# LuxGraph/Lux

Hardware: AMD Instinct MI355X
Metric: GTEPS (higher is better)
Workload: dtype fp32; 1 GPU; model=pagerank, graph=rmat27, nv=134217728, ne=2147483648, parallelism=graph-partition x1

## Files before the change

lux_amd/_native_gpu.py:

```python
import ctypes
import os

_DIR = os.path.dirname(os.path.abspath(__file__))
_PATH = os.path.join(_DIR, "liblux_gpu.so")

_lib = None


def lib():
    global _lib
    if _lib is None:
        if not os.path.exists(_PATH):
            raise RuntimeError(
                "liblux_gpu.so not built — run `python build.py --gpu` "
                "(the HIP extension is mandatory on GPU boxes; no fallback)")
        _lib = ctypes.CDLL(_PATH)
        _lib.lux_gpu_scan_partials_size.restype = ctypes.c_uint32
    return _lib


def dp(t):
    if t is None:
        return ctypes.c_void_p(0)
    if isinstance(t, int):
# ... 104 lines not shown
    lib().lux_gpu_build_bitmap(_u64(stream), _u32(vp), dp(snapshot),
                               dp(new_labels), dp(seg))


def d2s(stream, vp, row_left, dense_seg, sparse_seg):
    lib().lux_gpu_d2s(_u64(stream), _u32(vp), _u32(row_left), dp(dense_seg),
                      dp(sparse_seg))


def check(stream, is_min, vp, row_left, row_ptr_loc, col, labels, mistakes):
    lib().lux_gpu_check(_u64(stream), ctypes.c_int(is_min), _u32(vp),
                        _u32(row_left), dp(row_ptr_loc), dp(col), dp(labels),
                        dp(mistakes))


PULL_PR = 0
PULL_MIN = 1
PULL_MAX = 2


def pull_iter(stream, mode, n0, bin0, n1, bin1, n2, bin2, nbig, bin2v,
              row_ptr, col, oldv, newv, deg, row_left, init_rank,
              row_u32=0):
    lib().lux_gpu_pull_iter(_u64(stream), ctypes.c_int(mode), _u32(n0),
                            dp(bin0), _u32(n1), dp(bin1), _u32(n2), dp(bin2),
                            _u32(nbig), dp(bin2v), dp(row_ptr),
                            ctypes.c_int(row_u32), dp(col),
                            dp(oldv), dp(newv), dp(deg), _u32(row_left),
                            ctypes.c_float(init_rank))


def blocked_count(stream, ep, col, row_ptr_loc, vp, bounds, nb, counts,
                  lo=0, hi=0xFFFFFFFF):
    lib().lux_gpu_blocked_count(_u64(stream), _u64(ep), dp(col),
                                dp(row_ptr_loc), _u32(vp), dp(bounds),
                                ctypes.c_int(nb), _u32(lo), _u32(hi),
                                dp(counts))


def blocked_scatter(stream, ep, col, row_ptr_loc, vp, bounds, nb, cursor,
                    out_col, lo=0, hi=0xFFFFFFFF):
    lib().lux_gpu_blocked_scatter(_u64(stream), _u64(ep), dp(col),
                                  dp(row_ptr_loc), _u32(vp), dp(bounds),
                                  ctypes.c_int(nb), _u32(lo), _u32(hi),
                                  dp(cursor), dp(out_col))


def pull_finish_pr(stream, vp, newv, deg, row_left, init_rank):
    lib().lux_gpu_pull_finish_pr(_u64(stream), _u32(vp), dp(newv), dp(deg),
                                 _u32(row_left), ctypes.c_float(init_rank))


def pull_active_flags(stream, vp, row_ptr, flags):
    lib().lux_gpu_pull_active_flags(_u64(stream), _u32(vp), dp(row_ptr),
                                    dp(flags))


def pull_active_list(stream, vp, flags, ends, active):
    lib().lux_gpu_pull_active_list(_u64(stream), _u32(vp), dp(flags),
                                   dp(ends), dp(active))


def pull_build_slots(stream, n, bin_, row_ptr, row_u32, ends, cidx, rng):
    lib().lux_gpu_pull_build_slots(_u64(stream), _u32(n), dp(bin_),
                                   dp(row_ptr), ctypes.c_int(row_u32),
                                   dp(ends), dp(cidx), dp(rng))


def pull_build_hub_slots(stream, n2, bin2, row_ptr, row_u32, ends, cidx,
                         rng):
    lib().lux_gpu_pull_build_hub_slots(_u64(stream), _u32(n2), dp(bin2),
                                       dp(row_ptr), ctypes.c_int(row_u32),
                                       dp(ends), dp(cidx), dp(rng))


def pull_slots_iter(stream, n0, cidx0, rng0, n1, cidx1, rng1, n2, cidx2,
                    rng2, col, oldv, acc):
    lib().lux_gpu_pull_slots_iter(_u64(stream), _u32(n0), dp(cidx0),
                                  dp(rng0), _u32(n1), dp(cidx1), dp(rng1),
                                  _u32(n2), dp(cidx2), dp(rng2), dp(col),
                                  dp(oldv), dp(acc))


def pull_finish_pr_active(stream, na, active, acc, out, deg, row_left,
                          init_rank):
    lib().lux_gpu_pull_finish_pr_active(_u64(stream), _u32(na), dp(active),
                                        dp(acc), dp(out), dp(deg),
                                        _u32(row_left),
                                        ctypes.c_float(init_rank))


def pull_fill_inactive_pr(stream, vp, row_ptr, out, deg, row_left,
                          init_rank):
    lib().lux_gpu_pull_fill_inactive_pr(_u64(stream), _u32(vp), dp(row_ptr),
                                        dp(out), dp(deg), _u32(row_left),
                                        ctypes.c_float(init_rank))


def cf_als_iter(stream, n0, bin0, n1, bin1, n2, bin2, nbig, bin2v, hubidx,
                gram_scratch, rhs_scratch, row_ptr, col, w, oldv, newv,
                row_left, K, oldv_bf=None):
    lib().lux_gpu_cf_als_iter(
        _u64(stream), _u32(n0), dp(bin0), _u32(n1), dp(bin1), _u32(n2),
        dp(bin2), _u32(nbig), dp(bin2v), dp(hubidx), dp(gram_scratch),
        dp(rhs_scratch), dp(row_ptr), dp(col), dp(w), dp(oldv), dp(oldv_bf),
        dp(newv), _u32(row_left), ctypes.c_int(K))


def frontier_expand(stream, old_dense, in_row_left, in_count, old_seg,
                    qlabels, labels_repair, push_row_ptr, items, counter,
                    max_items):
    lib().lux_gpu_frontier_expand(
        _u64(stream), ctypes.c_int(old_dense), _u32(in_row_left),
        _u32(in_count), dp(old_seg), dp(qlabels), dp(labels_repair),
        dp(push_row_ptr), dp(items), dp(counter), _u32(max_items))


def frontier_expand_auto(stream, verts, in_row_left, seg, qlabels,
                         labels_repair, push_row_ptr, items, counter,
                         max_items):
    lib().lux_gpu_frontier_expand_auto(
        _u64(stream), _u32(verts), _u32(in_row_left), dp(seg), dp(qlabels),
        dp(labels_repair), dp(push_row_ptr), dp(items), dp(counter),
        _u32(max_items))


def frontier_fixup(stream, vp, row_left, capacity, built_dense, snapshot,
                   labels_part, deg_part, new_seg, annex, tmp_seg, meta,
                   item_counter, max_items):
    lib().lux_gpu_frontier_fixup(
        _u64(stream), _u32(vp), _u32(row_left), _u32(capacity),
        ctypes.c_int(built_dense), dp(snapshot), dp(labels_part),
        dp(deg_part), dp(new_seg), dp(annex), dp(tmp_seg), dp(meta),
        dp(item_counter), _u32(max_items))


def push_chunk_scatter(stream, is_min, new_dense, items, counter, max_items,
                       push_row_ptr, push_col, old_labels, snapshot,
                       new_labels, my_row_left, new_seg, capacity,
                       visited_bits=None):
    lib().lux_gpu_push_chunk_scatter(
        _u64(stream), ctypes.c_int(is_min), ctypes.c_int(new_dense),
        dp(items), dp(counter), _u32(max_items), dp(push_row_ptr),
        dp(push_col), dp(old_labels), dp(snapshot), dp(new_labels),
        _u32(my_row_left), dp(new_seg), _u32(capacity), dp(visited_bits))


def publish_labels_guarded(stream, vp, meta, labels_part, labels_slice):
    lib().lux_gpu_publish_labels_guarded(_u64(stream), _u32(vp), dp(meta),
                                         dp(labels_part), dp(labels_slice))


def bits_from_labels(stream, vp, labels, bits):
    lib().lux_gpu_bits_from_labels(_u64(stream), _u32(vp), dp(labels),
                                   dp(bits))


def uf_union_star(stream, nv, star, parent):
    lib().lux_gpu_uf_union_star(_u64(stream), _u32(nv), dp(star), dp(parent))


def uf_flatten(stream, nv, parent, labels):
    lib().lux_gpu_uf_flatten(_u64(stream), _u32(nv), dp(parent), dp(labels))


def uf_union_binned(stream, n0, bin0, n1, bin1, n2, bin2, row_ptr, col,
# ... 16 lines not shown
```

lux_amd/engine.py:

```python

import torch

from . import _native_gpu as ng
from . import dist as dx

U32 = torch.int32
U64 = torch.int64
F32 = torch.float32


def _stream():
    return torch.cuda.current_stream().cuda_stream


LLC_BLOCK_SHIFT = 23


def _bins_for(row_ptr, vp, ep, device, compact=False):
    s = _stream()
    bin0 = torch.empty(max(vp, 1), dtype=U32, device=device)
    bin1 = torch.empty(max(vp, 1), dtype=U32, device=device)
    nbig_max = max(min(vp, ep // 2048 + 1), 1)
    n2_max = ep // 8192 + nbig_max + 1
    bin2 = torch.empty(n2_max * 2, dtype=U32, device=device)
    bin2v = torch.empty(nbig_max, dtype=U32, device=device)
    counters = torch.zeros(4, dtype=U32, device=device)
    ng.build_bins(s, vp, row_ptr, bin0, bin1, bin2, bin2v, counters)
    c = counters.cpu()
    n0, n1, n2, nbig = int(c[0]), int(c[1]), int(c[2]), int(c[3])
    if compact:
        bin0 = bin0[:max(n0, 1)].clone()
        bin1 = bin1[:max(n1, 1)].clone()
        bin2 = bin2[:max(n2 * 2, 1)].clone()
        bin2v = bin2v[:max(nbig, 1)].clone()
    return n0, n1, n2, nbig, bin0, bin1, bin2, bin2v


def run_pull_sweeps(part, mode, oldv, newv, deg, init_rank, subset=None):
    s = _stream()
    blocks = getattr(part, "blocks", None)
    if blocks:
        for blk in blocks:
            if subset == "local" and not blk["local"]:
                continue
            if subset == "remote" and blk["local"]:
                continue
            if isinstance(subset, tuple) and subset[0] == "peer" \
                    and blk.get("owner") != subset[1]:
                continue
            ng.pull_iter(s, mode, blk["n0"], blk["bin0"], blk["n1"],
                         blk["bin1"], blk["n2"], blk["bin2"], blk["nbig"],
                         blk["bin2v"], blk["row_ptr"], blk["col"], oldv,
                         newv, deg, part.row_left, init_rank,
                         row_u32=blk.get("row_u32", 0))
    else:
        assert subset is None, "subset sweeps need the blocked CSC"
        ng.pull_iter(s, mode, part.n0, part.bin0, part.n1, part.bin1,
                     part.n2, part.bin2, part.nbig, part.bin2v, part.row_ptr,
                     part.col, oldv, newv, deg, part.row_left, init_rank)


def run_pull_slots_sweeps(part, oldv, acc):
    s = _stream()
    for src in part.slot_srcs:
        ng.pull_slots_iter(s, src["n0"], src["cidx0"], src["rng0"],
                           src["n1"], src["cidx1"], src["rng1"], src["n2"],
                           src["cidx2"], src["rng2"], src["col"], oldv, acc)


def seed_pull(part, mode, oldv, newv):
    if mode == ng.PULL_PR:
        newv.zero_()
    else:
        newv.copy_(oldv.narrow(0, part.row_left, part.vp))


def run_pull(part, mode, oldv, newv, deg, init_rank, seed=True):
    if seed:
        seed_pull(part, mode, oldv, newv)
    run_pull_sweeps(part, mode, oldv, newv, deg, init_rank)
    if mode == ng.PULL_PR:
        ng.pull_finish_pr(_stream(), part.vp, newv, deg, part.row_left,
                          init_rank)


def partition_bounds(col_end, ne, nparts):
    nv = col_end.numel()
    cap = (ne + nparts - 1) // nparts
    targets = torch.tensor(
        [min(cap * (p + 1), ne) for p in range(nparts)], dtype=U64,
        device=col_end.device)
    cuts = torch.searchsorted(col_end, targets, right=True)
    cuts = cuts.cpu().tolist()
    row_left, row_right = [], []
    v = 0
    for p in range(nparts):
        rl = v
        rr = max(cuts[p] - 1, rl) if p < nparts - 1 else nv - 1
        rr = min(rr, nv - 1)
        if rl >= nv:
            row_left.append(1)
            row_right.append(0)
            continue
        row_left.append(rl)
        row_right.append(rr)
        v = rr + 1
    return row_left, row_right


class DeviceCSC:

    n_users = None

    def __init__(self, nv, ne, col_end, src, weight=None):
        self.nv, self.ne = nv, ne
        self.col_end, self.src, self.weight = col_end, src, weight

    @classmethod
    def rmat(cls, scale, ne, seed=1, device="cuda", sym=False):
        nv = 1 << scale
        s = _stream()
        npairs = ne // 2 if sym else ne
        esrc = torch.empty(npairs, dtype=U32, device=device)
        edst = torch.empty(npairs, dtype=U32, device=device)
        ng.rmat_edges(s, seed, scale, npairs, esrc, edst)
        if sym:
            esrc, edst = (torch.cat([esrc, edst]), torch.cat([edst, esrc]))
        g = cls._from_device_edges(nv, npairs * 2 if sym else ne, esrc,
                                   edst, None, device)
        return g

    @classmethod
    def rmat_folded(cls, nv, ne, seed=1, device="cuda", sym=False):
        scale = 0
        while (1 << scale) < nv:
            scale += 1
        s = _stream()
        npairs = ne // 2 if sym else ne
        esrc = torch.empty(npairs, dtype=U32, device=device)
        edst = torch.empty(npairs, dtype=U32, device=device)
        ng.rmat_edges_folded(s, seed, scale, nv, npairs, esrc, edst)
        if sym:
            esrc, edst = (torch.cat([esrc, edst]), torch.cat([edst, esrc]))
        return cls._from_device_edges(nv, npairs * 2 if sym else ne, esrc,
                                      edst, None, device)

# ... 213 lines not shown
            return
        (self.n0, self.n1, self.n2, self.nbig, self.bin0, self.bin1,
         self.bin2, self.bin2v) = _bins_for(self.row_ptr, self.vp, self.ep,
                                            self.device)

    def pull_bounds(self, shift):
        bounds = set(range(0, self.nv, 1 << shift)) | {self.nv}
        if self.nparts > 1 and self.vp > 0:
            for q in range(self.nparts):
                if self.verts_all[q]:
                    bounds |= {self.row_left_all[q],
                               self.row_right_all[q] + 1}
        return sorted(bounds)

    def prepare_pull(self, force_shift=None):
        self.build_bins()
        if getattr(self, "blocks", None) is not None:
            return
        shift = force_shift if force_shift is not None else int(
            __import__("os").environ.get("LUX_BLOCK_SHIFT", LLC_BLOCK_SHIFT))
        if force_shift is None and torch.cuda.is_available() \
                and self.vp > 0:
            free, _total = torch.cuda.mem_get_info(self.device)
            while shift < 30:
                sb = len(self.pull_bounds(shift)) - 1
                need = 12 * sb * self.vp + 4 * self.ep
                if need < free * 0.85:
                    break
                shift += 1
        bounds = self.pull_bounds(shift)
        if self.ep == 0 or len(bounds) <= 2:
            self.blocks = None
            return
        if force_shift is None and self.nv <= (1 << shift) \
                and self.nparts == 1:
            self.blocks = None
            return
        self.build_blocked(bounds)

    def prepare_pull_slots(self):
        if getattr(self, "slot_srcs", None) is not None:
            return True
        self.prepare_pull()
        if not self.blocks and self.ep >= (1 << 32):
            return False
        device, s, vp = self.device, _stream(), self.vp
        before = torch.cuda.memory_allocated(device)
        self.na = 0
        self.active = torch.empty(1, dtype=U32, device=device)
        self.slot_srcs = []
        if vp == 0 or self.ep == 0:
            self.slot_bytes = 0
            return True
        flags = torch.empty(vp, dtype=U32, device=device)
        ng.pull_active_flags(s, vp, self.row_ptr, flags)
        ends = torch.empty(vp, dtype=U64, device=device)
        partials = torch.empty(ng.scan_partials_size(vp), dtype=U64,
                               device=device)
        ng.scan_end_offsets(s, vp, flags, ends, partials)
        self.na = int(ends[vp - 1].item())
        self.active = torch.empty(max(self.na, 1), dtype=U32, device=device)
        ng.pull_active_list(s, vp, flags, ends, self.active)
        if self.blocks:
            srcs = self.blocks
        else:
            srcs = [dict(row_ptr=self.row_ptr, row_u32=0, col=self.col,
                         n0=self.n0, n1=self.n1, n2=self.n2, bin0=self.bin0,
                         bin1=self.bin1, bin2=self.bin2)]
        for src in srcs:
            for k, build in (("0", ng.pull_build_slots),
                             ("1", ng.pull_build_slots),
                             ("2", ng.pull_build_hub_slots)):
                n = src["n" + k]
                cidx = torch.empty(max(n, 1), dtype=U32, device=device)
                rng = torch.empty(max(2 * n, 2), dtype=U32, device=device)
                build(s, n, src["bin" + k], src["row_ptr"],
                      src.get("row_u32", 0), ends, cidx, rng)
                src["cidx" + k], src["rng" + k] = cidx, rng
            self.slot_srcs.append(src)
        torch.cuda.synchronize()
        del flags, ends, partials
        self.slot_bytes = torch.cuda.memory_allocated(device) - before
        return True

    def build_blocked(self, bounds):
        import os
        device = self.device
        s = _stream()
        vp, ep = self.vp, self.ep
        sb = len(bounds) - 1
        cap = int(os.environ.get("LUX_BLOCK_GROUP_SLOTS", "0") or 0)
        if not cap and torch.cuda.is_available():
            free, _total = torch.cuda.mem_get_info(device)
            cap = int(max(free - 4 * ep - (2 << 30), 1 << 30) * 0.85) // 12
        bpg = sb if not cap else max(1, min(sb, cap // max(vp, 1)))
        blk_col = torch.empty(max(ep, 1), dtype=U32, device=device)
        self.blocks = []
        global_begin = 0
        for g0 in range(0, sb, bpg):
            g1 = min(sb, g0 + bpg)
            nb = g1 - g0
            slots = nb * vp
            bounds_g = torch.tensor(bounds[g0:g1 + 1], dtype=U32,
                                    device=device)
            counts = torch.zeros(slots, dtype=U32, device=device)
            ng.blocked_count(s, ep, self.col, self.row_ptr, vp, bounds_g,
                             nb + 1, counts, lo=bounds[g0], hi=bounds[g1])
            cursor = torch.zeros(slots + 1, dtype=U64, device=device)
            partials = torch.empty(ng.scan_partials_size(slots), dtype=U64,
                                   device=device)
            ng.scan_end_offsets(s, slots, counts,
                                cursor.narrow(0, 1, slots), partials)
            torch.cuda.synchronize()
            del counts, partials
            torch.cuda.empty_cache()
            if global_begin:
                cursor += global_begin
            ng.blocked_scatter(s, ep, self.col, self.row_ptr, vp, bounds_g,
                               nb + 1, cursor.narrow(0, 0, slots), blk_col,
                               lo=bounds[g0], hi=bounds[g1])
            ends = cursor.narrow(0, 0, slots)
            begin = global_begin
            for b in range(nb):
                end = int(ends[(b + 1) * vp - 1].item())
                if end == begin:
                    continue
                row_ptr_b = torch.empty(vp + 1, dtype=U64, device=device)
                ng.local_row_ptr(s, vp, begin, ends.narrow(0, b * vp, vp),
                                 row_ptr_b)
                col_b = blk_col.narrow(0, begin, end - begin)
                n0, n1, n2, nbig, b0, b1, b2, b2v = _bins_for(
                    row_ptr_b, vp, end - begin, device, compact=True)
                row32 = torch.empty(vp + 1, dtype=U32, device=device)
                ng.u64_to_u32(s, vp + 1, row_ptr_b, row32)
                del row_ptr_b
                gb = g0 + b
                owner = -1
                if self.nparts > 1:
                    for q in range(self.nparts):
                        if self.verts_all[q] \
                                and bounds[gb] >= self.row_left_all[q] \
                                and bounds[gb + 1] \
                                <= self.row_right_all[q] + 1:
                            owner = q
                            break
                local = self.nparts > 1 and owner == self.p
                self.blocks.append(dict(row_ptr=row32, row_u32=1, col=col_b,
                                        n0=n0, n1=n1, n2=n2, nbig=nbig,
                                        bin0=b0, bin1=b1, bin2=b2,
                                        bin2v=b2v, local=local,
                                        owner=owner))
                begin = end
            global_begin = int(ends[slots - 1].item())
            del ends, cursor
        self._blk_col = blk_col


def _maybe_halo(part):
    if dx.world_size() <= 1 or part.vp == 0:
        return None
    from .halo import HaloExchange
    h = HaloExchange(part.nv, part.row_left_all, part.verts_all, part.p,
                     part.col)
    return h if h.worth_it() else None


def _publish_async(engine, my_slice):
    p = engine.part
    if engine.halo is not None:
        return engine.halo.publish_async(engine.old, my_slice)
    return dx.all_gather_slices_async(engine.old, my_slice, p.verts_all,
                                      p.row_left_all, my_index=p.p)


def _wait_handle(engine):
    h = engine._handle
    engine._handle = None
    if h is None:
        return
    if isinstance(h, list):
        for _q, w in h:
            w.wait()
    else:
        h.wait()


def _finalize_full(engine):
    _wait_handle(engine)
    if engine.halo is None:
        return
    p = engine.part
    dx.all_gather_slices(engine.old,
                         engine.old.narrow(0, p.row_left, p.vp),
                         p.verts_all, p.row_left_all, my_index=p.p)


class PagerankEngine:

    def __init__(self, part: GraphPart):
        self.part = part
        device = part.device
        s = _stream()
        deg = torch.zeros(part.nv, dtype=U32, device=device)
        ng.hist_u32(s, part.ep, part.col, deg)
        dx.all_reduce_sum_(deg)
        self.deg = deg
        part.prepare_pull()
        rank0 = 1.0 / part.nv
        degf = deg.to(F32)
        self.old = torch.where(deg == 0, torch.full_like(degf, rank0),
                               rank0 / degf.clamp(min=1.0))
        self.init_rank = (1.0 - 0.15) / part.nv
        import os
        self._slots = (dx.world_size() == 1
                       and os.environ.get("LUX_PULL_SLOTS", "1") != "0"
                       and part.prepare_pull_slots())
        if self._slots:
            self.acc = torch.empty(max(part.na, 1), dtype=F32,
                                   device=device)
            self.new_part = None
            self._inactive_done = False
        else:
            self.new_part = torch.empty(part.vp, dtype=F32, device=device)
        self.cur_part = self.old.narrow(0, part.row_left,
                                        part.vp).clone()
        self._handle = None
        self.halo = _maybe_halo(part)
        self._graph = None
        self._steps = 0

    def _pipelined(self):
        p = self.part
        return dx.world_size() > 1 and p.blocks is not None and p.vp > 0

    def _step_body(self):
        p = self.part
        if self._slots:
            self.acc.zero_()
            run_pull_slots_sweeps(p, self.old, self.acc)
            ng.pull_finish_pr_active(_stream(), p.na, p.active, self.acc,
                                     self.old, self.deg, p.row_left,
                                     self.init_rank)
            return
        run_pull(p, ng.PULL_PR, self.old, self.new_part, self.deg,
                 self.init_rank)
        self.old.narrow(0, p.row_left, p.vp).copy_(self.new_part)

    def _step_single(self):
        import os
        if self._graph is not None:
            self._graph.replay()
            return
        if self._steps >= 2 and os.environ.get("LUX_HIPGRAPH", "1") \
                == "1" and not os.environ.get("LUX_SYNC_CHECK"):
            try:
                g = torch.cuda.CUDAGraph()
                with torch.cuda.graph(g):
                    self._step_body()
                self._graph = g
                self._graph.replay()
                return
            except Exception as e:
                print(f"[lux] hipGraph capture disabled: {e}")
                os.environ["LUX_HIPGRAPH"] = "0"
        self._step_body()

    def step(self):
        p = self.part
        if not self._pipelined():
            if dx.world_size() > 1:
                run_pull(p, ng.PULL_PR, self.old, self.new_part, self.deg,
                         self.init_rank)
                _publish_async(self, self.new_part).wait()
                return
            self._steps += 1
            self._step_single()
            if self._slots and not self._inactive_done:
                ng.pull_fill_inactive_pr(_stream(), p.vp, p.row_ptr,
                                         self.old, self.deg, p.row_left,
                                         self.init_rank)
                self._inactive_done = True
            return
        self.new_part.zero_()
        local_base = self.cur_part.data_ptr() - p.row_left * 4
        run_pull_sweeps(p, ng.PULL_PR, local_base, self.new_part, self.deg,
                        self.init_rank, subset="local")
        if isinstance(self._handle, list):
            for q, w in self._handle:
                w.wait()
                run_pull_sweeps(p, ng.PULL_PR, self.old, self.new_part,
                                self.deg, self.init_rank,
                                subset=("peer", q))
            run_pull_sweeps(p, ng.PULL_PR, self.old, self.new_part,
                            self.deg, self.init_rank, subset=("peer", -1))
            self._handle = None
        else:
            if self._handle is not None:
                self._handle.wait()
                self._handle = None
            run_pull_sweeps(p, ng.PULL_PR, self.old, self.new_part,
                            self.deg, self.init_rank, subset="remote")
        ng.pull_finish_pr(_stream(), p.vp, self.new_part, self.deg,
                          p.row_left, self.init_rank)
        self.cur_part, self.new_part = self.new_part, self.cur_part
        if self.halo is None:
            self._handle = dx.all_gather_slices_per_peer(
                self.old, self.cur_part, p.verts_all, p.row_left_all,
                my_index=p.p)
        else:
            self._handle = _publish_async(self, self.cur_part)

    def finalize(self):
        _finalize_full(self)

    def ranks(self):
        _wait_handle(self)
        return self.old


class LabelPullEngine:

    def __init__(self, part: GraphPart, mode, init_labels):
# ... 72 lines not shown
```

src/gpu/pull.hip:

```cpp
#include "gpu_common.h"

namespace lux {

constexpr V_ID T1 = 32;
constexpr V_ID T2 = 2048;
constexpr V_ID CHUNK_EDGES = 8192;

enum PullMode { PR_SUM = 0, LAB_MIN = 1, LAB_MAX = 2, CF_SGD = 3 };


__global__ void build_bins_kernel(V_ID vp, const E_ID* row_ptr,
                                  V_ID* bin0, V_ID* bin1, uint2* bin2,
                                  V_ID* bin2v, uint32_t* counters) {
  __shared__ uint32_t lcnt[4], lbase[4];
  uint64_t stride = (uint64_t)blockDim.x * gridDim.x;
  for (uint64_t tile = (uint64_t)blockIdx.x * blockDim.x; tile < vp;
       tile += stride) {
    uint64_t v = tile + threadIdx.x;
    if (threadIdx.x < 4) lcnt[threadIdx.x] = 0;
    __syncthreads();
    int my_bin = -1;
    uint32_t lpos = 0, nchunks = 0, lpos_c = 0;
    if (v < vp) {
      E_ID deg = row_ptr[v + 1] - row_ptr[v];
// ... 198 lines not shown
      continue;
    E_ID b, e;
    src.range(i, v, b, e);
    T acc = gather_range<M>(oldv, a.col, b + lane, e, WAVE);
    acc = V::reduce_wave(acc);
    if (lane == 0)
      store_result<M>(&newv[v], acc);
  }
}

template <PullMode M, typename Src>
__device__ __forceinline__ void pull_chunk_role(uint32_t blk, uint32_t nblk,
                                                uint32_t n2, const Src& src,
                                                const PullArgs& a) {
  using V = Val<M>;
  using T = typename V::T;
  __shared__ T lds[BLOCK / WAVE];
  const T* oldv = (const T*)a.oldv;
  T* newv = (T*)a.newv;
  for (uint32_t i = blk; i < n2; i += nblk) {
    uint32_t chunk = 0;
    V_ID v = src.row(i, chunk);
    if (V::SKIP_SETTLED && oldv[a.row_left + v] != (T)INF_LABEL)
      continue;
    E_ID b, e;
    src.range(i, v, chunk, b, e);
    T acc = gather_range<M>(oldv, a.col, b + threadIdx.x, e, blockDim.x);
    int lane = threadIdx.x & (WAVE - 1);
    int wid = threadIdx.x >> 6;
    acc = V::reduce_wave(acc);
    if (lane == 0) lds[wid] = acc;
    __syncthreads();
    if (threadIdx.x == 0) {
      acc = lds[0];
      for (int w = 1; w < (int)(blockDim.x / WAVE); w++)
        acc = V::comb(acc, lds[w]);
      V::atom(&newv[v], acc);
    }
    __syncthreads();
  }
}

template <PullMode M, typename RowT>
__global__ void pull_thread_kernel(uint32_t n0, const V_ID* bin0,
                                   PullArgs a) {
  pull_thread_role<M>(blockIdx.x, gridDim.x, n0,
                      TableRows<RowT>{bin0, (const RowT*)a.row_ptr}, a);
}

template <PullMode M, typename RowT>
__global__ void pull_wave_kernel(uint32_t n1, const V_ID* bin1, PullArgs a) {
  pull_wave_role<M>(blockIdx.x, gridDim.x, n1,
                    TableRows<RowT>{bin1, (const RowT*)a.row_ptr}, a);
}

template <PullMode M, typename RowT>
__global__ void pull_chunk_kernel(uint32_t n2, const uint2* bin2,
                                  PullArgs a) {
  pull_chunk_role<M>(blockIdx.x, gridDim.x, n2,
                     TableChunks<RowT>{bin2, (const RowT*)a.row_ptr}, a);
}

struct SlotBins {
  uint32_t n0, n1, n2;
  uint32_t g1, g2;
  const V_ID *cidx0, *cidx1, *cidx2;
  const uint2 *rng0, *rng1, *rng2;
};

template <PullMode M>
__global__ void __launch_bounds__(BLOCK)
    pull_slots_kernel(SlotBins s, PullArgs a) {
  uint32_t blk = blockIdx.x;
  if (blk < s.g2) {
    pull_chunk_role<M>(blk, s.g2, s.n2, SlotRows{s.cidx2, s.rng2}, a);
  } else if (blk < s.g2 + s.g1) {
    pull_wave_role<M>(blk - s.g2, s.g1, s.n1, SlotRows{s.cidx1, s.rng1}, a);
  } else {
    pull_thread_role<M>(blk - s.g2 - s.g1, gridDim.x - s.g2 - s.g1, s.n0,
                        SlotRows{s.cidx0, s.rng0}, a);
  }
}


__global__ void pull_active_flags_kernel(V_ID vp, const E_ID* row_ptr,
                                         uint32_t* flags) {
  uint64_t stride = (uint64_t)blockDim.x * gridDim.x;
  for (uint64_t v = blockIdx.x * (uint64_t)blockDim.x + threadIdx.x; v < vp;
       v += stride)
    flags[v] = row_ptr[v + 1] != row_ptr[v];
}

__global__ void pull_active_list_kernel(V_ID vp, const uint32_t* flags,
                                        const E_ID* ends, V_ID* active) {
  uint64_t stride = (uint64_t)blockDim.x * gridDim.x;
  for (uint64_t v = blockIdx.x * (uint64_t)blockDim.x + threadIdx.x; v < vp;
       v += stride)
    if (flags[v]) active[ends[v] - 1] = (V_ID)v;
}

template <typename RowT>
__global__ void pull_build_slots_kernel(uint32_t n, const V_ID* bin,
                                        const RowT* row_ptr, const E_ID* ends,
                                        V_ID* cidx, uint2* rng) {
  uint64_t stride = (uint64_t)blockDim.x * gridDim.x;
  for (uint64_t i = blockIdx.x * (uint64_t)blockDim.x + threadIdx.x; i < n;
       i += stride) {
    V_ID v = bin[i];
    cidx[i] = (V_ID)(ends[v] - 1);
    rng[i] = make_uint2((uint32_t)row_ptr[v], (uint32_t)row_ptr[v + 1]);
  }
}

template <typename RowT>
__global__ void pull_build_hub_slots_kernel(uint32_t n2, const uint2* bin2,
                                            const RowT* row_ptr,
                                            const E_ID* ends, V_ID* cidx,
                                            uint2* rng) {
  TableChunks<RowT> t{bin2, row_ptr};
  uint64_t stride = (uint64_t)blockDim.x * gridDim.x;
  for (uint64_t i = blockIdx.x * (uint64_t)blockDim.x + threadIdx.x; i < n2;
       i += stride) {
    uint32_t chunk;
    V_ID v = t.row(i, chunk);
    E_ID b, e;
    t.range(i, v, chunk, b, e);
    cidx[i] = (V_ID)(ends[v] - 1);
    rng[i] = make_uint2((uint32_t)b, (uint32_t)e);
  }
}


template <PullMode M, typename RowT>
static void pull_iter(hipStream_t s, uint32_t n0, const V_ID* bin0,
                      uint32_t n1, const V_ID* bin1, uint32_t n2,
                      const uint2* bin2, uint32_t nbig, const V_ID* bin2v,
                      const PullArgs& a) {
  if (nbig) {
    hipLaunchKernelGGL((pull_chunk_kernel<M, RowT>),
                       dim3(n2 > MAX_GRID ? MAX_GRID : n2), dim3(BLOCK), 0, s,
                       n2, bin2, a);
  }
  if (n1)
    hipLaunchKernelGGL((pull_wave_kernel<M, RowT>),
                       dim3(grid_for((uint64_t)n1 * WAVE)), dim3(BLOCK), 0, s,
                       n1, bin1, a);
  if (n0)
    hipLaunchKernelGGL((pull_thread_kernel<M, RowT>), dim3(grid_for(n0)),
                       dim3(BLOCK), 0, s, n0, bin0, a);
}

__device__ __forceinline__ float finish_pr(float sum, V_ID d,
                                           float init_rank) {
  float pr = init_rank + PR_ALPHA * sum;
  return d != 0 ? pr / (float)d : pr;
}

__global__ void pull_finish_pr_kernel(V_ID vp, float* newv,
                                      const V_ID* deg, V_ID row_left,
                                      float init_rank) {
  uint64_t stride = (uint64_t)blockDim.x * gridDim.x;
  for (uint64_t v = blockIdx.x * (uint64_t)blockDim.x + threadIdx.x; v < vp;
       v += stride)
    newv[v] = finish_pr(newv[v], deg[row_left + v], init_rank);
}

__global__ void pull_finish_pr_active_kernel(V_ID na, const V_ID* active,
                                             const float* acc, float* out,
                                             const V_ID* deg, V_ID row_left,
                                             float init_rank) {
  uint64_t stride = (uint64_t)blockDim.x * gridDim.x;
  for (uint64_t i = blockIdx.x * (uint64_t)blockDim.x + threadIdx.x; i < na;
       i += stride) {
    uint64_t g = (uint64_t)row_left + active[i];
    out[g] = finish_pr(acc[i], deg[g], init_rank);
  }
}

__global__ void pull_fill_inactive_pr_kernel(V_ID vp, const E_ID* row_ptr,
                                             float* out, const V_ID* deg,
                                             V_ID row_left,
                                             float init_rank) {
  uint64_t stride = (uint64_t)blockDim.x * gridDim.x;
  for (uint64_t v = blockIdx.x * (uint64_t)blockDim.x + threadIdx.x; v < vp;
       v += stride) {
    if (row_ptr[v + 1] != row_ptr[v]) continue;
    uint64_t g = (uint64_t)row_left + v;
    out[g] = finish_pr(0.0f, deg[g], init_rank);
  }
}

}


using namespace lux;

extern "C" {

void lux_gpu_build_bins(uint64_t stream, uint32_t vp, const E_ID* row_ptr,
                        V_ID* bin0, V_ID* bin1, uint2* bin2, V_ID* bin2v,
                        uint32_t* counters ) {
  hipStream_t s = (hipStream_t)stream;
  hipLaunchKernelGGL(build_bins_kernel, dim3(grid_for(vp)), dim3(BLOCK), 0, s,
                     vp, row_ptr, bin0, bin1, bin2, bin2v, counters);
  LUX_POST_LAUNCH(stream);
}

void lux_gpu_pull_iter(uint64_t stream, int mode, uint32_t n0,
                       const V_ID* bin0, uint32_t n1, const V_ID* bin1,
                       uint32_t n2, const uint2* bin2, uint32_t nbig,
                       const V_ID* bin2v, const void* row_ptr, int row_u32,
                       const V_ID* col, const void* oldv, void* newv,
                       const V_ID* deg, V_ID row_left, float init_rank) {
  hipStream_t s = (hipStream_t)stream;
// ... 2 lines not shown
  switch (mode) {
    case 0: LUX_PI(PR_SUM); break;
    case 1: LUX_PI(LAB_MIN); break;
    case 2: LUX_PI(LAB_MAX); break;
  }
#undef LUX_PI
  LUX_POST_LAUNCH(stream);
}

void lux_gpu_pull_finish_pr(uint64_t stream, V_ID vp, float* newv,
                            const V_ID* deg, V_ID row_left,
                            float init_rank) {
  hipStream_t s = (hipStream_t)stream;
  hipLaunchKernelGGL(pull_finish_pr_kernel, dim3(grid_for(vp)), dim3(BLOCK),
                     0, s, vp, newv, deg, row_left, init_rank);
  LUX_POST_LAUNCH(stream);
}


void lux_gpu_pull_active_flags(uint64_t stream, V_ID vp, const E_ID* row_ptr,
                               uint32_t* flags) {
  hipLaunchKernelGGL(pull_active_flags_kernel, dim3(grid_for(vp)),
                     dim3(BLOCK), 0, (hipStream_t)stream, vp, row_ptr, flags);
  LUX_POST_LAUNCH(stream);
}

void lux_gpu_pull_active_list(uint64_t stream, V_ID vp, const uint32_t* flags,
                              const E_ID* ends, V_ID* active) {
  hipLaunchKernelGGL(pull_active_list_kernel, dim3(grid_for(vp)), dim3(BLOCK),
                     0, (hipStream_t)stream, vp, flags, ends, active);
  LUX_POST_LAUNCH(stream);
}

void lux_gpu_pull_build_slots(uint64_t stream, uint32_t n, const V_ID* bin,
                              const void* row_ptr, int row_u32,
                              const E_ID* ends, V_ID* cidx, uint2* rng) {
  if (!n) return;
  hipStream_t s = (hipStream_t)stream;
  if (row_u32)
    hipLaunchKernelGGL(pull_build_slots_kernel<uint32_t>, dim3(grid_for(n)),
                       dim3(BLOCK), 0, s, n, bin, (const uint32_t*)row_ptr,
                       ends, cidx, rng);
  else
    hipLaunchKernelGGL(pull_build_slots_kernel<uint64_t>, dim3(grid_for(n)),
                       dim3(BLOCK), 0, s, n, bin, (const uint64_t*)row_ptr,
                       ends, cidx, rng);
  LUX_POST_LAUNCH(stream);
}

void lux_gpu_pull_build_hub_slots(uint64_t stream, uint32_t n2,
                                  const uint2* bin2, const void* row_ptr,
                                  int row_u32, const E_ID* ends, V_ID* cidx,
                                  uint2* rng) {
  if (!n2) return;
  hipStream_t s = (hipStream_t)stream;
  if (row_u32)
    hipLaunchKernelGGL(pull_build_hub_slots_kernel<uint32_t>,
                       dim3(grid_for(n2)), dim3(BLOCK), 0, s, n2, bin2,
                       (const uint32_t*)row_ptr, ends, cidx, rng);
  else
    hipLaunchKernelGGL(pull_build_hub_slots_kernel<uint64_t>,
                       dim3(grid_for(n2)), dim3(BLOCK), 0, s, n2, bin2,
                       (const uint64_t*)row_ptr, ends, cidx, rng);
  LUX_POST_LAUNCH(stream);
}

void lux_gpu_pull_slots_iter(uint64_t stream, uint32_t n0, const V_ID* cidx0,
                             const uint2* rng0, uint32_t n1,
                             const V_ID* cidx1, const uint2* rng1,
                             uint32_t n2, const V_ID* cidx2,
                             const uint2* rng2, const V_ID* col,
                             const float* oldv, float* acc) {
  uint32_t g2 = n2 ? (n2 > (uint32_t)MAX_GRID ? MAX_GRID : n2) : 0;
  uint32_t g1 = n1 ? grid_for((uint64_t)n1 * WAVE) : 0;
  uint32_t g0 = n0 ? grid_for(n0) : 0;
  if (g0 + g1 + g2 == 0) return;
  SlotBins sb{n0, n1, n2, g1, g2, cidx0, cidx1, cidx2, rng0, rng1, rng2};
  PullArgs a{nullptr, col, oldv, acc, nullptr, 0, 0.0f};
  hipLaunchKernelGGL(pull_slots_kernel<PR_SUM>, dim3(g0 + g1 + g2),
                     dim3(BLOCK), 0, (hipStream_t)stream, sb, a);
  LUX_POST_LAUNCH(stream);
}

void lux_gpu_pull_finish_pr_active(uint64_t stream, V_ID na,
                                   const V_ID* active, const float* acc,
                                   float* out, const V_ID* deg, V_ID row_left,
                                   float init_rank) {
  if (!na) return;
  hipLaunchKernelGGL(pull_finish_pr_active_kernel, dim3(grid_for(na)),
                     dim3(BLOCK), 0, (hipStream_t)stream, na, active, acc,
                     out, deg, row_left, init_rank);
  LUX_POST_LAUNCH(stream);
}

void lux_gpu_pull_fill_inactive_pr(uint64_t stream, V_ID vp,
                                   const E_ID* row_ptr, float* out,
                                   const V_ID* deg, V_ID row_left,
                                   float init_rank) {
  if (!vp) return;
  hipLaunchKernelGGL(pull_fill_inactive_pr_kernel, dim3(grid_for(vp)),
                     dim3(BLOCK), 0, (hipStream_t)stream, vp, row_ptr, out,
                     deg, row_left, init_rank);
  LUX_POST_LAUNCH(stream);
}

}
```

src/include/lux/gpu_api.h:

```cpp
#pragma once
#include <cstdint>

#include "types.h"

#ifndef __HIP_PLATFORM_AMD__
struct lux_uint2 { uint32_t x, y; };
#else
using lux_uint2 = uint2;
#endif

extern "C" {

void lux_gpu_rmat_edges(uint64_t stream, uint64_t seed, int scale,
                        uint64_t ne, lux::V_ID* src, lux::V_ID* dst);
void lux_gpu_rmat_edges_folded(uint64_t stream, uint64_t seed, int scale,
                               lux::V_ID nv, uint64_t ne, lux::V_ID* src,
                               lux::V_ID* dst);
void lux_gpu_bipartite_edges(uint64_t stream, uint64_t seed,
                             lux::V_ID n_users, lux::V_ID n_items,
                             uint64_t ne, lux::V_ID* src, lux::V_ID* dst,
                             lux::WeightType* w);
void lux_gpu_hist_u32(uint64_t stream, uint64_t n, const lux::V_ID* ids,
                      uint32_t* hist);
void lux_gpu_rmat_edges_chunk(uint64_t stream, uint64_t seed, int scale,
                              uint64_t e0, uint64_t ne, lux::V_ID* src,
                              lux::V_ID* dst);
void lux_gpu_rmat_edges_folded_chunk(uint64_t stream, uint64_t seed,
                                     int scale, lux::V_ID nv, uint64_t e0,
                                     uint64_t ne, lux::V_ID* src,
                                     lux::V_ID* dst);
void lux_gpu_bipartite_edges_chunk(uint64_t stream, uint64_t seed,
                                   lux::V_ID n_users, lux::V_ID n_items,
                                   uint64_t e0, uint64_t ne, lux::V_ID* src,
                                   lux::V_ID* dst, lux::WeightType* w);
void lux_gpu_slice_scatter(uint64_t stream, uint64_t n, const lux::V_ID* src,
                           const lux::V_ID* dst, const lux::WeightType* w,
                           lux::V_ID rl, lux::V_ID rr,
                           unsigned long long* cursor, lux::V_ID* out_col,
                           lux::WeightType* out_w);
uint32_t lux_gpu_scan_partials_size(uint64_t n);
void lux_gpu_scan_end_offsets(uint64_t stream, uint64_t n,
                              const uint32_t* in, lux::E_ID* out_end,
                              unsigned long long* partials);
void lux_gpu_u64_to_u32(uint64_t stream, uint64_t n,
                        const unsigned long long* in, uint32_t* out);
void lux_gpu_edges_to_csc(uint64_t stream, uint32_t nv, uint64_t ne,
                          const lux::V_ID* src, const lux::V_ID* dst,
                          const lux::WeightType* w, lux::E_ID* col_end,
                          lux::V_ID* out_src, lux::WeightType* out_w,
                          uint32_t* hist, unsigned long long* cursor,
                          unsigned long long* partials);
void lux_gpu_local_row_ptr(uint64_t stream, uint32_t vp, lux::E_ID col_left,
                           const lux::E_ID* col_end_slice,
                           lux::E_ID* row_ptr_loc);
void lux_gpu_blocked_count(uint64_t stream, uint64_t ep, const lux::V_ID* col,
                           const lux::E_ID* row_ptr_loc, lux::V_ID vp,
                           const lux::V_ID* bounds, int nb, lux::V_ID lo,
                           lux::V_ID hi, uint32_t* counts);
void lux_gpu_blocked_scatter(uint64_t stream, uint64_t ep,
                             const lux::V_ID* col,
                             const lux::E_ID* row_ptr_loc, lux::V_ID vp,
                             const lux::V_ID* bounds, int nb, lux::V_ID lo,
                             lux::V_ID hi, unsigned long long* cursor,
                             lux::V_ID* out_col);

void lux_gpu_build_bins(uint64_t stream, uint32_t vp,
                        const lux::E_ID* row_ptr, lux::V_ID* bin0,
                        lux::V_ID* bin1, lux_uint2* bin2, lux::V_ID* bin2v,
                        uint32_t* counters);
void lux_gpu_pull_iter(uint64_t stream, int mode, uint32_t n0,
                       const lux::V_ID* bin0, uint32_t n1,
                       const lux::V_ID* bin1, uint32_t n2,
                       const lux_uint2* bin2, uint32_t nbig,
                       const lux::V_ID* bin2v, const void* row_ptr,
                       int row_u32, const lux::V_ID* col, const void* oldv,
                       void* newv, const lux::V_ID* deg, lux::V_ID row_left,
                       float init_rank);
void lux_gpu_pull_finish_pr(uint64_t stream, lux::V_ID vp, float* newv,
                            const lux::V_ID* deg, lux::V_ID row_left,
                            float init_rank);
void lux_gpu_pull_active_flags(uint64_t stream, lux::V_ID vp,
                               const lux::E_ID* row_ptr, uint32_t* flags);
void lux_gpu_pull_active_list(uint64_t stream, lux::V_ID vp,
                              const uint32_t* flags, const lux::E_ID* ends,
                              lux::V_ID* active);
void lux_gpu_pull_build_slots(uint64_t stream, uint32_t n,
                              const lux::V_ID* bin, const void* row_ptr,
                              int row_u32, const lux::E_ID* ends,
                              lux::V_ID* cidx, lux_uint2* rng);
void lux_gpu_pull_build_hub_slots(uint64_t stream, uint32_t n2,
                                  const lux_uint2* bin2, const void* row_ptr,
                                  int row_u32, const lux::E_ID* ends,
                                  lux::V_ID* cidx, lux_uint2* rng);
void lux_gpu_pull_slots_iter(uint64_t stream, uint32_t n0,
                             const lux::V_ID* cidx0, const lux_uint2* rng0,
                             uint32_t n1, const lux::V_ID* cidx1,
                             const lux_uint2* rng1, uint32_t n2,
                             const lux::V_ID* cidx2, const lux_uint2* rng2,
                             const lux::V_ID* col, const float* oldv,
                             float* acc);
void lux_gpu_pull_finish_pr_active(uint64_t stream, lux::V_ID na,
                                   const lux::V_ID* active, const float* acc,
                                   float* out, const lux::V_ID* deg,
                                   lux::V_ID row_left, float init_rank);
void lux_gpu_pull_fill_inactive_pr(uint64_t stream, lux::V_ID vp,
                                   const lux::E_ID* row_ptr, float* out,
                                   const lux::V_ID* deg, lux::V_ID row_left,
                                   float init_rank);

void lux_gpu_csr_scatter(uint64_t stream, uint64_t ep, const lux::V_ID* col,
                         const lux::E_ID* row_ptr_loc, lux::V_ID vp,
                         lux::V_ID row_left, unsigned long long* cursor,
                         lux::V_ID* push_col);
void lux_gpu_frontier_expand(uint64_t stream, int old_dense,
                             lux::V_ID in_row_left, lux::V_ID in_count,
                             const uint8_t* old_seg,
                             const uint32_t* qlabels ,
                             uint32_t* labels_repair ,
                             const lux::E_ID* push_row_ptr,
                             lux_uint2* items, uint32_t* counter,
                             uint32_t max_items);
void lux_gpu_frontier_expand_auto(uint64_t stream, lux::V_ID verts,
                                  lux::V_ID in_row_left, const uint8_t* seg,
                                  const uint32_t* qlabels,
                                  uint32_t* labels_repair,
                                  const lux::E_ID* push_row_ptr,
                                  lux_uint2* items, uint32_t* counter,
                                  uint32_t max_items);
void lux_gpu_frontier_fixup(uint64_t stream, lux::V_ID vp,
                            lux::V_ID row_left, lux::V_ID capacity,
                            int built_dense, const uint32_t* snapshot,
                            const uint32_t* labels_part,
                            const uint32_t* deg_part, uint8_t* new_seg,
                            uint32_t* annex, uint8_t* tmp_seg,
                            uint32_t* meta,
                            const uint32_t* item_counter ,
                            uint32_t max_items);
void lux_gpu_push_chunk_scatter(uint64_t stream, int is_min, int new_dense,
                                const lux_uint2* items,
                                const uint32_t* counter, uint32_t max_items,
                                const lux::E_ID* push_row_ptr,
                                const lux::V_ID* push_col,
                                const uint32_t* old_labels,
                                const uint32_t* snapshot,
                                uint32_t* new_labels, lux::V_ID my_row_left,
                                uint8_t* new_seg, lux::V_ID capacity,
                                uint32_t* visited_bits );
void lux_gpu_bits_from_labels(uint64_t stream, lux::V_ID vp,
                              const uint32_t* labels, uint32_t* bits);

void lux_gpu_build_bitmap(uint64_t stream, lux::V_ID vp,
                          const uint32_t* snapshot,
                          const uint32_t* new_labels, uint8_t* seg);
void lux_gpu_d2s(uint64_t stream, lux::V_ID vp, lux::V_ID row_left,
                 const uint8_t* dense_seg, uint8_t* sparse_seg);
void lux_gpu_publish_labels_guarded(uint64_t stream, lux::V_ID vp,
                                    const uint32_t* meta,
                                    const uint32_t* labels_part,
                                    uint32_t* labels_slice);
void lux_gpu_check(uint64_t stream, int is_min, lux::V_ID vp,
                   lux::V_ID row_left, const lux::E_ID* row_ptr_loc,
                   const lux::V_ID* col, const uint32_t* labels,
                   unsigned long long* mistakes);

void lux_gpu_cf_seed(uint64_t stream, uint64_t n, const float* oldv,
                     float* newv);
void lux_gpu_cf_iter(uint64_t stream, uint32_t n0, const lux::V_ID* bin0,
                     uint32_t n1, const lux::V_ID* bin1, uint32_t n2,
                     const lux_uint2* bin2, uint32_t nbig,
                     const lux::V_ID* bin2v, const lux::E_ID* row_ptr,
                     const lux::V_ID* col, const lux::WeightType* w,
                     const float* oldv, float* newv, lux::V_ID row_left,
                     int K);

void lux_gpu_count_diff(uint64_t stream, uint64_t n, const uint32_t* a,
                        const uint32_t* b, unsigned long long* out);
void lux_gpu_uf_union_binned(uint64_t stream, uint32_t n0,
                             const lux::V_ID* bin0, uint32_t n1,
                             const lux::V_ID* bin1, uint32_t n2,
                             const lux_uint2* bin2, const lux::E_ID* row_ptr,
                             const lux::V_ID* col, lux::V_ID row_left,
                             lux::V_ID* parent, const uint32_t* gbits);
void lux_gpu_uf_union_kth(uint64_t stream, lux::V_ID vp,
// ... 22 lines not shown
```

Before: 130.8 GTEPS.

## Stream low-degree pull rows through packed edge tiles with wave-local LDS reduction

Adds a one-time preprocessing step that copies the edge lists of low-degree (bin0) rows into a contiguous packed column array and cuts them into tiles of up to 512 edges spanning at most 64 rows. A new stream role in the fused slots kernel has each wave load a whole tile with coalesced, unrolled gathers into LDS, then segment-sums per row from shared memory, prefetching the next tile's bounds. This replaces per-row slot handling for small rows, aiming at better memory-level parallelism and fewer underfilled wave iterations. The cost is an extra copy of the bin0 column data in device memory and a more complex tiling and prefetch scheme, and it is enabled by default.

```diff
diff --git a/lux_amd/_native_gpu.py b/lux_amd/_native_gpu.py
--- a/lux_amd/_native_gpu.py
+++ b/lux_amd/_native_gpu.py
@@ -210,6 +210,33 @@
                                   dp(oldv), dp(acc))
 
 
+def pull_slot_counts(stream, n, rng, cnt):
+    lib().lux_gpu_pull_slot_counts(_u64(stream), _u32(n), dp(rng), dp(cnt))
+
+
+def pull_stream_copy(stream, n0, rng0, off0, col, scol0):
+    lib().lux_gpu_pull_stream_copy(_u64(stream), _u32(n0), dp(rng0),
+                                   dp(off0), dp(col), dp(scol0))
+
+
+def pull_stream_tile_counts(stream, n0, off0, cnt):
+    lib().lux_gpu_pull_stream_tile_counts(_u64(stream), _u32(n0), dp(off0),
+                                          dp(cnt))
+
+
+def pull_stream_tile_fill(stream, n0, off0, ends, tile0):
+    lib().lux_gpu_pull_stream_tile_fill(_u64(stream), _u32(n0), dp(off0),
+                                        dp(ends), dp(tile0))
+
+
+def pull_slots_stream_iter(stream, n0, cidx0, nt, tile0, off0, scol0, n1,
+                           cidx1, rng1, n2, cidx2, rng2, col, oldv, acc):
+    lib().lux_gpu_pull_slots_stream_iter(
+        _u64(stream), _u32(n0), dp(cidx0), _u32(nt), dp(tile0), dp(off0),
+        dp(scol0), _u32(n1), dp(cidx1), dp(rng1), _u32(n2), dp(cidx2),
+        dp(rng2), dp(col), dp(oldv), dp(acc))
+
+
 def pull_finish_pr_active(stream, na, active, acc, out, deg, row_left,
                           init_rank):
     lib().lux_gpu_pull_finish_pr_active(_u64(stream), _u32(na), dp(active),
diff --git a/lux_amd/engine.py b/lux_amd/engine.py
--- a/lux_amd/engine.py
+++ b/lux_amd/engine.py
@@ -14,6 +14,8 @@
 
 
 LLC_BLOCK_SHIFT = 23
+
+PULL_STREAM_DEFAULT = "1"
 
 
 def _bins_for(row_ptr, vp, ep, device, compact=False):
@@ -60,8 +62,24 @@
                      part.col, oldv, newv, deg, part.row_left, init_rank)
 
 
-def run_pull_slots_sweeps(part, oldv, acc):
+def pull_stream_enabled():
+    import os
+    return os.environ.get("LUX_PULL_STREAM", PULL_STREAM_DEFAULT) != "0"
+
+
+def run_pull_slots_sweeps(part, oldv, acc, stream=None):
     s = _stream()
+    if stream is None:
+        stream = pull_stream_enabled()
+    if stream:
+        part.prepare_pull_stream()
+        for src in part.slot_srcs:
+            ng.pull_slots_stream_iter(
+                s, src["n0"], src["cidx0"], src["nt"], src["tile0"],
+                src["off0"], src["scol0"], src["n1"], src["cidx1"],
+                src["rng1"], src["n2"], src["cidx2"], src["rng2"],
+                src["col"], oldv, acc)
+        return
     for src in part.slot_srcs:
         ng.pull_slots_iter(s, src["n0"], src["cidx0"], src["rng0"],
                            src["n1"], src["cidx1"], src["rng1"], src["n2"],
@@ -441,6 +459,41 @@
         del flags, ends, partials
         self.slot_bytes = torch.cuda.memory_allocated(device) - before
         return True
+
+    def prepare_pull_stream(self):
+        if getattr(self, "stream_bytes", None) is not None:
+            return
+        device, s = self.device, _stream()
+        before = torch.cuda.memory_allocated(device)
+        for src in self.slot_srcs:
+            n0 = src["n0"]
+            if not n0:
+                src["nt"] = 0
+                src["off0"] = src["scol0"] = src["tile0"] = None
+                continue
+            cnt = torch.empty(n0, dtype=U32, device=device)
+            ng.pull_slot_counts(s, n0, src["rng0"], cnt)
+            ends = torch.empty(n0, dtype=U64, device=device)
+            partials = torch.empty(ng.scan_partials_size(n0), dtype=U64,
+                                   device=device)
+            ng.scan_end_offsets(s, n0, cnt, ends, partials)
+            off0 = torch.zeros(n0 + 1, dtype=U32, device=device)
+            ng.u64_to_u32(s, n0, ends, off0.narrow(0, 1, n0))
+            scol0 = torch.empty(int(ends[n0 - 1].item()), dtype=U32,
+                                device=device)
+            ng.pull_stream_copy(s, n0, src["rng0"], off0, src["col"], scol0)
+            ngroups = (n0 + 63) // 64
+            ng.pull_stream_tile_counts(s, n0, off0, cnt)
+            ng.scan_end_offsets(s, ngroups, cnt, ends, partials)
+            nt = int(ends[ngroups - 1].item())
+            tile0 = torch.empty(nt + 1, dtype=U32, device=device)
+            ng.pull_stream_tile_fill(s, n0, off0, ends, tile0)
+            src["nt"], src["off0"], src["scol0"], src["tile0"] = \
+                nt, off0, scol0, tile0
+        torch.cuda.synchronize()
+        cnt = ends = partials = None
+        self.stream_bytes = torch.cuda.memory_allocated(device) - before
+        self.slot_bytes += self.stream_bytes
 
     def build_blocked(self, bounds):
         import os
@@ -574,6 +627,9 @@
         self._slots = (dx.world_size() == 1
                        and os.environ.get("LUX_PULL_SLOTS", "1") != "0"
                        and part.prepare_pull_slots())
+        self._stream_role = bool(self._slots) and pull_stream_enabled()
+        if self._stream_role:
+            part.prepare_pull_stream()
         if self._slots:
             self.acc = torch.empty(max(part.na, 1), dtype=F32,
                                    device=device)
@@ -596,7 +652,8 @@
         p = self.part
         if self._slots:
             self.acc.zero_()
-            run_pull_slots_sweeps(p, self.old, self.acc)
+            run_pull_slots_sweeps(p, self.old, self.acc,
+                                  stream=self._stream_role)
             ng.pull_finish_pr_active(_stream(), p.na, p.active, self.acc,
                                      self.old, self.deg, p.row_left,
                                      self.init_rank)
diff --git a/src/gpu/pull.hip b/src/gpu/pull.hip
--- a/src/gpu/pull.hip
+++ b/src/gpu/pull.hip
@@ -304,6 +304,112 @@
   }
 }
 
+constexpr uint32_t TILE_EDGES = 512;
+constexpr uint32_t TILE_GROUP = WAVE;
+
+struct SlotStream {
+  uint32_t nt;
+  const uint32_t* tile0;
+  const uint32_t* off0;
+  const V_ID* scol0;
+};
+
+__device__ __forceinline__ float lds_range_sum(const float* v, uint32_t j,
+                                               uint32_t e) {
+  float a0 = 0.0f, a1 = 0.0f, a2 = 0.0f, a3 = 0.0f;
+  for (; j + 3 < e; j += 4) {
+    a0 = a0 + v[j];
+    a1 = a1 + v[j + 1];
+    a2 = a2 + v[j + 2];
+    a3 = a3 + v[j + 3];
+  }
+  for (; j < e; j++) a0 = a0 + v[j];
+  return (a0 + a1) + (a2 + a3);
+}
+
+template <PullMode M>
+__device__ __forceinline__ void pull_stream_role(uint32_t blk, uint32_t nblk,
+                                                 const SlotStream& st,
+                                                 const V_ID* cidx0,
+                                                 const PullArgs& a) {
+  static_assert(M == PR_SUM, "stream role: float sums only");
+  constexpr uint32_t NW = BLOCK / WAVE;
+  __shared__ float vals[NW][TILE_EDGES];
+  const float* oldv = (const float*)a.oldv;
+  float* acc = (float*)a.newv;
+  uint32_t lane = threadIdx.x & (WAVE - 1);
+  uint32_t wid = __builtin_amdgcn_readfirstlane(threadIdx.x >> 6);
+  float* v = vals[wid];
+  uint64_t nwaves = (uint64_t)nblk * NW;
+  uint64_t t = (uint64_t)blk * NW + wid;
+  if (t >= st.nt) return;
+  uint32_t s0 = st.tile0[t], s1 = st.tile0[t + 1];
+  uint32_t e0 = st.off0[s0], e1 = st.off0[s1];
+  for (;;) {
+    uint64_t tn = t + nwaves;
+    bool more = tn < st.nt;
+    uint32_t s0n = 0, s1n = 0, e0n = 0, e1n = 0;
+    if (more) {
+      s0n = st.tile0[tn];
+      s1n = st.tile0[tn + 1];
+    }
+    uint32_t rb = 0, re = 0;
+    V_ID ci = 0;
+    float prev = 0.0f;
+    bool row = lane < s1 - s0;
+    if (row) {
+      rb = st.off0[s0 + lane] - e0;
+      re = st.off0[s0 + lane + 1] - e0;
+      ci = cidx0[s0 + lane];
+      prev = acc[ci];
+    }
+    for (uint32_t base = e0 + lane; base < e1; base += 4 * WAVE) {
+      uint32_t i0 = base, i1 = base + WAVE, i2 = base + 2 * WAVE,
+               i3 = base + 3 * WAVE;
+      bool p1 = i1 < e1, p2 = i2 < e1, p3 = i3 < e1;
+      V_ID c0 = st.scol0[i0];
+      V_ID c1 = p1 ? st.scol0[i1] : 0;
+      V_ID c2 = p2 ? st.scol0[i2] : 0;
+      V_ID c3 = p3 ? st.scol0[i3] : 0;
+      float x0 = oldv[c0];
+      float x1 = p1 ? oldv[c1] : 0.0f;
+      float x2 = p2 ? oldv[c2] : 0.0f;
+      float x3 = p3 ? oldv[c3] : 0.0f;
+      v[i0 - e0] = x0;
+      if (p1) v[i1 - e0] = x1;
+      if (p2) v[i2 - e0] = x2;
+      if (p3) v[i3 - e0] = x3;
+    }
+    if (more) {
+      e0n = st.off0[s0n];
+      e1n = st.off0[s1n];
+    }
+    __builtin_amdgcn_fence(__ATOMIC_RELEASE, "wavefront");
+    __builtin_amdgcn_wave_barrier();
+    __builtin_amdgcn_fence(__ATOMIC_ACQUIRE, "wavefront");
+    if (row) acc[ci] = Val<M>::comb(lds_range_sum(v, rb, re), prev);
+    __builtin_amdgcn_fence(__ATOMIC_RELEASE, "wavefront");
+    __builtin_amdgcn_wave_barrier();
+    if (!more) break;
+    t = tn;
+    s0 = s0n, s1 = s1n, e0 = e0n, e1 = e1n;
+  }
+}
+
+template <PullMode M>
+__global__ void __launch_bounds__(BLOCK)
+    pull_slots_stream_kernel(SlotBins s, SlotStream st, PullArgs a) {
+  uint32_t blk = blockIdx.x;
+  if (blk < s.g2) {
+    pull_chunk_role<M>(blk, s.g2, s.n2, SlotRows{s.cidx2, s.rng2}, a);
+  } else if (blk < s.g2 + s.g1) {
+    pull_wave_role<M>(blk - s.g2, s.g1, s.n1, SlotRows{s.cidx1, s.rng1}, a);
+  } else {
+    pull_stream_role<M>(blk - s.g2 - s.g1, gridDim.x - s.g2 - s.g1, st,
+                        s.cidx0, a);
+  }
+}
+
 
 __global__ void pull_active_flags_kernel(V_ID vp, const E_ID* row_ptr,
                                          uint32_t* flags) {
@@ -352,6 +458,68 @@
   }
 }
 
+
+__global__ void pull_slot_counts_kernel(uint32_t n, const uint2* rng,
+                                        uint32_t* cnt) {
+  uint64_t stride = (uint64_t)blockDim.x * gridDim.x;
+  for (uint64_t i = blockIdx.x * (uint64_t)blockDim.x + threadIdx.x; i < n;
+       i += stride) {
+    uint2 r = rng[i];
+    cnt[i] = r.y - r.x;
+  }
+}
+
+__global__ void pull_stream_copy_kernel(uint32_t n0, const uint2* rng0,
+                                        const uint32_t* off0,
+                                        const V_ID* col, V_ID* scol0) {
+  uint64_t stride = (uint64_t)blockDim.x * gridDim.x;
+  for (uint64_t i = blockIdx.x * (uint64_t)blockDim.x + threadIdx.x; i < n0;
+       i += stride) {
+    uint2 r = rng0[i];
+    uint32_t o = off0[i];
+    for (uint32_t j = r.x; j < r.y; j++) scol0[o + (j - r.x)] = col[j];
+  }
+}
+
+__device__ __forceinline__ uint32_t cut_tile_group(uint64_t g, uint32_t n0,
+                                                   const uint32_t* off0,
+                                                   uint32_t* out) {
+  uint64_t s = g * TILE_GROUP;
+  uint64_t send = s + TILE_GROUP < n0 ? s + TILE_GROUP : n0;
+  uint32_t begin = off0[s], nt = 1;
+  if (out) out[0] = (uint32_t)s;
+  for (uint64_t i = s; i < send; i++) {
+    if (off0[i + 1] - begin > TILE_EDGES) {
+      begin = off0[i];
+      if (out) out[nt] = (uint32_t)i;
+      nt++;
+    }
+  }
+  return nt;
+}
+
+__global__ void pull_stream_tile_counts_kernel(uint32_t n0,
+                                               const uint32_t* off0,
+                                               uint32_t* cnt) {
+  uint64_t ngroups = ((uint64_t)n0 + TILE_GROUP - 1) / TILE_GROUP;
+  uint64_t stride = (uint64_t)blockDim.x * gridDim.x;
+  for (uint64_t g = blockIdx.x * (uint64_t)blockDim.x + threadIdx.x;
+       g < ngroups; g += stride)
+    cnt[g] = cut_tile_group(g, n0, off0, nullptr);
+}
+
+__global__ void pull_stream_tile_fill_kernel(uint32_t n0,
+                                             const uint32_t* off0,
+                                             const E_ID* ends,
+                                             uint32_t* tile0) {
+  uint64_t ngroups = ((uint64_t)n0 + TILE_GROUP - 1) / TILE_GROUP;
+  uint64_t stride = (uint64_t)blockDim.x * gridDim.x;
+  for (uint64_t g = blockIdx.x * (uint64_t)blockDim.x + threadIdx.x;
+       g < ngroups; g += stride) {
+    cut_tile_group(g, n0, off0, tile0 + (g ? ends[g - 1] : 0));
+    if (g == ngroups - 1) tile0[ends[g]] = n0;
+  }
+}
 
 template <PullMode M, typename RowT>
 static void pull_iter(hipStream_t s, uint32_t n0, const V_ID* bin0,
@@ -520,6 +688,62 @@
   LUX_POST_LAUNCH(stream);
 }
 
+
+void lux_gpu_pull_slot_counts(uint64_t stream, uint32_t n, const uint2* rng,
+                              uint32_t* cnt) {
+  if (!n) return;
+  hipLaunchKernelGGL(pull_slot_counts_kernel, dim3(grid_for(n)), dim3(BLOCK),
+                     0, (hipStream_t)stream, n, rng, cnt);
+  LUX_POST_LAUNCH(stream);
+}
+
+void lux_gpu_pull_stream_copy(uint64_t stream, uint32_t n0, const uint2* rng0,
+                              const uint32_t* off0, const V_ID* col,
+                              V_ID* scol0) {
+  if (!n0) return;
+  hipLaunchKernelGGL(pull_stream_copy_kernel, dim3(grid_for(n0)), dim3(BLOCK),
+                     0, (hipStream_t)stream, n0, rng0, off0, col, scol0);
+  LUX_POST_LAUNCH(stream);
+}
+
+void lux_gpu_pull_stream_tile_counts(uint64_t stream, uint32_t n0,
+                                     const uint32_t* off0, uint32_t* cnt) {
+  if (!n0) return;
+  uint64_t ngroups = ((uint64_t)n0 + TILE_GROUP - 1) / TILE_GROUP;
+  hipLaunchKernelGGL(pull_stream_tile_counts_kernel, dim3(grid_for(ngroups)),
+                     dim3(BLOCK), 0, (hipStream_t)stream, n0, off0, cnt);
+  LUX_POST_LAUNCH(stream);
+}
+
+void lux_gpu_pull_stream_tile_fill(uint64_t stream, uint32_t n0,
+                                   const uint32_t* off0, const E_ID* ends,
+                                   uint32_t* tile0) {
+  if (!n0) return;
+  uint64_t ngroups = ((uint64_t)n0 + TILE_GROUP - 1) / TILE_GROUP;
+  hipLaunchKernelGGL(pull_stream_tile_fill_kernel, dim3(grid_for(ngroups)),
+                     dim3(BLOCK), 0, (hipStream_t)stream, n0, off0, ends,
+                     tile0);
+  LUX_POST_LAUNCH(stream);
+}
+
+void lux_gpu_pull_slots_stream_iter(
+    uint64_t stream, uint32_t n0, const V_ID* cidx0, uint32_t nt,
+    const uint32_t* tile0, const uint32_t* off0, const V_ID* scol0,
+    uint32_t n1, const V_ID* cidx1, const uint2* rng1, uint32_t n2,
+    const V_ID* cidx2, const uint2* rng2, const V_ID* col, const float* oldv,
+    float* acc) {
+  uint32_t g2 = n2 ? (n2 > (uint32_t)MAX_GRID ? MAX_GRID : n2) : 0;
+  uint32_t g1 = n1 ? grid_for((uint64_t)n1 * WAVE) : 0;
+  uint32_t g0 = n0 && nt ? grid_for((uint64_t)nt * WAVE) : 0;
+  if (g0 + g1 + g2 == 0) return;
+  SlotBins sb{n0, n1, n2, g1, g2, cidx0, cidx1, cidx2, nullptr, rng1, rng2};
+  SlotStream st{g0 ? nt : 0, tile0, off0, scol0};
+  PullArgs a{nullptr, col, oldv, acc, nullptr, 0, 0.0f};
+  hipLaunchKernelGGL(pull_slots_stream_kernel<PR_SUM>, dim3(g0 + g1 + g2),
+                     dim3(BLOCK), 0, (hipStream_t)stream, sb, st, a);
+  LUX_POST_LAUNCH(stream);
+}
+
 void lux_gpu_pull_finish_pr_active(uint64_t stream, V_ID na,
                                    const V_ID* active, const float* acc,
                                    float* out, const V_ID* deg, V_ID row_left,
diff --git a/src/include/lux/gpu_api.h b/src/include/lux/gpu_api.h
--- a/src/include/lux/gpu_api.h
+++ b/src/include/lux/gpu_api.h
@@ -99,6 +99,22 @@
                              const lux::V_ID* cidx2, const lux_uint2* rng2,
                              const lux::V_ID* col, const float* oldv,
                              float* acc);
+void lux_gpu_pull_slot_counts(uint64_t stream, uint32_t n,
+                              const lux_uint2* rng, uint32_t* cnt);
+void lux_gpu_pull_stream_copy(uint64_t stream, uint32_t n0,
+                              const lux_uint2* rng0, const uint32_t* off0,
+                              const lux::V_ID* col, lux::V_ID* scol0);
+void lux_gpu_pull_stream_tile_counts(uint64_t stream, uint32_t n0,
+                                     const uint32_t* off0, uint32_t* cnt);
+void lux_gpu_pull_stream_tile_fill(uint64_t stream, uint32_t n0,
+                                   const uint32_t* off0,
+                                   const lux::E_ID* ends, uint32_t* tile0);
+void lux_gpu_pull_slots_stream_iter(
+    uint64_t stream, uint32_t n0, const lux::V_ID* cidx0, uint32_t nt,
+    const uint32_t* tile0, const uint32_t* off0, const lux::V_ID* scol0,
+    uint32_t n1, const lux::V_ID* cidx1, const lux_uint2* rng1, uint32_t n2,
+    const lux::V_ID* cidx2, const lux_uint2* rng2, const lux::V_ID* col,
+    const float* oldv, float* acc);
 void lux_gpu_pull_finish_pr_active(uint64_t stream, lux::V_ID na,
                                    const lux::V_ID* active, const float* acc,
                                    float* out, const lux::V_ID* deg,
```

Measured after the change: 138.6 GTEPS (median of 6 runs). 1.06x the previous value.
